# tammypi/flink-siddhi

Measured on AMD Instinct MI355X. Metric: matched-pattern events/sec (whole node) at 1/2/4/8 MI355X + % HBM roofline, higher is better.
Workload: dtype f64+int32+int64

## Files before the change

### flink-siddhi_amd/csrc/cf_kernels.hip

```cpp
#include <hip/hip_runtime.h>

#include "dev_common.h"
#include "kernels.h"
#include "vm.h"

namespace cep {

namespace {

constexpr uint16_t kNoB = 0xffff;
constexpr uint32_t kRolePB = 4;
constexpr int64_t kTolBias = 1ll << 31;
constexpr uint32_t kSkrAlive = 0x8000u;
constexpr int kCfStageBytes = (kCfTile / 8192 * 20 + 36) * 1024;

#ifdef CF_WAVESTAMP
#define CF_STAMP(i) do { } while (0)
#else
#define CF_STAMP(i)                                                                 \
  do {                                                                              \
    if (a.stamps && threadIdx.x == 0 && blockIdx.x < 4096)                          \
      a.stamps[(int64_t)blockIdx.x * 16 + (i)] = __builtin_amdgcn_s_memtime();      \
  } while (0)
#endif
// ... 276 lines not shown
  }
  lds_barrier();
  CF_STAMP(3);
  const uint32_t total = hist[NB];
  const uint32_t nreg = ATL ? hist[P] : total;
  const uint32_t words_t = nreg * RW + (total - nreg);
  const bool staged = words_t <= (uint32_t)(kStageRecs * RW);
  uint64_t* trecs = a.recs + tile * (int64_t)kCfTile * RW;
#pragma unroll
  for (int e = 0; e < E; ++e) {
    if (packed[e] == 0xffffffffu) continue;
    const uint32_t b = (packed[e] >> 13) & 0xfffu;
    const uint32_t role = packed[e] >> 25;
    const uint32_t slot = hist[b] + (packed[e] & 0x1fffu);
    const int64_t dts = (int64_t)tsv[e] - ts_base + (TOL ? kTolBias : 0);
    if (dts < 0) {
      if (TOL) set_err(a.err, ERR_TS_SPAN);
      else if (ATL) *(volatile uint32_t*)a.gate = a.gate_seq;
      else report_descent(a.rows, a.err);
    } else if (dts > 0xffffffffll) {
      set_err(a.err, ERR_TS_SPAN);
    }
    const uint64_t w0 = (uint64_t)(uint32_t)dts | ((uint64_t)(wave * 64 * E + 64 * e + lane) << 32) |
                        ((uint64_t)role << 45) | ((uint64_t)lkey[e] << 48);
    const uint64_t c0 = fc0[e], c1 = fc1[e];
    if (ATL && b >= (uint32_t)P) {
      const uint32_t wd = nreg * RW + (slot - nreg);
      if (staged) stage[wd] = w0;
      else trecs[wd] = w0;
      continue;
    }
    if (staged) {
      stage[slot * RW] = w0;
      if (NW > 0) stage[slot * RW + 1] = c0;
      if (NW > 1) stage[slot * RW + 2] = c1;
    } else {
      uint64_t* g = trecs + (int64_t)slot * RW;
      g[0] = w0;
      if (NW > 0) g[1] = c0;
      if (NW > 1) g[2] = c1;
    }
  }
  for (int i = tid; i <= NB; i += NT) a.tile_off[(int64_t)i * a.ntiles + tile] = (uint16_t)hist[i];
  if (staged) {
    lds_barrier();
    CF_STAMP(4);
    const int64_t words = (int64_t)words_t;
    for (int64_t w = 2 * tid; w < words; w += 2 * NT) {
      if (w + 1 < words) *(uint4*)(trecs + w) = *(const uint4*)(stage + w);
      else trecs[w] = stage[w];
    }
  }
  CF_STAMP(5);
}

#if !defined(CF_UNIT) || CF_UNIT == 1
constexpr int kCfRouteStage = 112 * 1024;
constexpr int kRouteSmallWorld = 8;
__global__ __launch_bounds__(kCfPartThreads, 1) void k_cfroute(CfRouteArgs ca) {
  constexpr int E = kCfItems, NT = kCfPartThreads, NWV = NT / 64;
  const RouteArgs& a = ca.r;
  const PatternArgs& p = a.pat;
  __shared__ uint32_t wcnt[NWV][kMaxWorld];
  __shared__ uint32_t obase[kMaxWorld + 1];
  __shared__ __attribute__((aligned(16))) uint64_t stage[kCfRouteStage / 8];
  const int tid = threadIdx.x, lane = tid & 63, wave = tid >> 6;
  const int world = a.world, wrw = a.wrw;
  const int64_t tile = blockIdx.x;
  for (int i = tid; i < NWV * kMaxWorld; i += NT) wcnt[i / kMaxWorld][i % kMaxWorld] = 0;

  const int64_t r0 = tile * kCfTile + (int64_t)wave * 64 * E + lane;
  const int64_t row0 = a.rows.row0 + r0;
  uint32_t valid = 0;
#pragma unroll
  for (int e = 0; e < E; ++e) valid |= (r0 + 64 * e < a.rows.n ? 1u : 0u) << e;
  uint64_t tsv[E], pv[kPref][E];
#pragma unroll
  for (int e = 0; e < E; ++e) tsv[e] = 0;
  uint32_t is_a = 0, role_a = 0, role_b = 0, role_g = 0;
  uint64_t fkey[E], fc0[E], fc1[E];
#pragma unroll
  for (int e = 0; e < E; ++e) fkey[e] = fc0[e] = fc1[e] = 0;
  if (valid) {
    uint32_t sb[E];
    cf_load_cols<E>(a.rows, ca.pref, ca.ts_slot, row0, valid, tsv, sb, pv);
    uint32_t is_b = 0;
#pragma unroll
    for (int e = 0; e < E; ++e) {
      if ((valid >> e) & 1u) {
        is_a |= ((int)sb[e] == p.a_stream ? 1u : 0u) << e;
        is_b |= ((int)sb[e] == p.b_stream ? 1u : 0u) << e;
      }
    }
    const uint32_t all = (1u << E) - 1u;
    if (is_a) role_a = is_a & (p.f_prog < 0 ? all : eval_terms_regs<E>(p.f_terms, ca.pref.f_slot, a.rows.cols, pv));
    if (is_b) {
      if (p.g_walk_prog >= 0) {
        role_b = is_b;
      } else {
        role_g = is_b & (p.g_raw_prog < 0 ? all : eval_terms_regs<E>(p.g_terms, ca.pref.g_slot, a.rows.cols, pv));
        role_b = p.tolerant ? is_b : role_g;
      }
    }
    if (p.nrec_a > 0 || p.nrec_b > 0)
      pick_carried<E>(pv, p.nrec_a > 0 ? ca.pref.reca_slot[0] : -1, p.nrec_b > 0 ? ca.pref.recb_slot[0] : -1,
                      is_a, fc0);
// ... 1126 lines not shown
  }
  const int np = a.pref.n <= 2 ? 2 : a.pref.n;
  switch (a.cf.nw * 8 + np) {
    case 0 * 8 + 2: hipLaunchKernelGGL((k_cfpart<0, false, 2, true>), g, b, dyn, s, a); break;
    case 0 * 8 + 3: hipLaunchKernelGGL((k_cfpart<0, false, 3, true>), g, b, dyn, s, a); break;
    case 0 * 8 + 4: hipLaunchKernelGGL((k_cfpart<0, false, 4, true>), g, b, dyn, s, a); break;
    case 1 * 8 + 2: hipLaunchKernelGGL((k_cfpart<1, false, 2, true>), g, b, dyn, s, a); break;
    case 1 * 8 + 3: hipLaunchKernelGGL((k_cfpart<1, false, 3, true>), g, b, dyn, s, a); break;
    case 1 * 8 + 4: hipLaunchKernelGGL((k_cfpart<1, false, 4, true>), g, b, dyn, s, a); break;
    case 2 * 8 + 2: hipLaunchKernelGGL((k_cfpart<2, false, 2, true>), g, b, dyn, s, a); break;
    case 2 * 8 + 3: hipLaunchKernelGGL((k_cfpart<2, false, 3, true>), g, b, dyn, s, a); break;
    default: hipLaunchKernelGGL((k_cfpart<2, false, 4, true>), g, b, dyn, s, a); break;
  }
}
#endif

template <int NW, bool ATL>
static void cf_part_local(const CfPartArgs& a, int64_t ntiles, hipStream_t s) {
  const int P = 1 << a.pat.buckets_log2;
  const size_t dyn = ((size_t)(P + a.nhot + 1) * 4 + 15) & ~(size_t)15;
  const dim3 g((unsigned)ntiles), b(kCfPartThreads);
  const int np = a.pref.n <= 2 ? 2 : a.pref.n;
  switch (np) {
    case 2: hipLaunchKernelGGL((k_cfpart<NW, false, 2, false, ATL>), g, b, dyn, s, a); break;
    case 3: hipLaunchKernelGGL((k_cfpart<NW, false, 3, false, ATL>), g, b, dyn, s, a); break;
    default: hipLaunchKernelGGL((k_cfpart<NW, false, 4, false, ATL>), g, b, dyn, s, a); break;
  }
}
void cf_part_et0(const CfPartArgs&, int64_t, hipStream_t);
void cf_part_et1(const CfPartArgs&, int64_t, hipStream_t);
void cf_part_et2(const CfPartArgs&, int64_t, hipStream_t);
void cf_part_atl0(const CfPartArgs&, int64_t, hipStream_t);
void cf_part_atl1(const CfPartArgs&, int64_t, hipStream_t);
void cf_part_atl2(const CfPartArgs&, int64_t, hipStream_t);
#if !defined(CF_UNIT) || CF_UNIT == 9
void cf_part_et0(const CfPartArgs& a, int64_t n, hipStream_t s) { cf_part_local<0, false>(a, n, s); }
#endif
#if !defined(CF_UNIT) || CF_UNIT == 10
void cf_part_et1(const CfPartArgs& a, int64_t n, hipStream_t s) { cf_part_local<1, false>(a, n, s); }
#endif
#if !defined(CF_UNIT) || CF_UNIT == 11
void cf_part_et2(const CfPartArgs& a, int64_t n, hipStream_t s) { cf_part_local<2, false>(a, n, s); }
#endif
#if !defined(CF_UNIT) || CF_UNIT == 12
void cf_part_atl0(const CfPartArgs& a, int64_t n, hipStream_t s) { cf_part_local<0, true>(a, n, s); }
#endif
#if !defined(CF_UNIT) || CF_UNIT == 13
void cf_part_atl1(const CfPartArgs& a, int64_t n, hipStream_t s) { cf_part_local<1, true>(a, n, s); }
#endif
#if !defined(CF_UNIT) || CF_UNIT == 14
void cf_part_atl2(const CfPartArgs& a, int64_t n, hipStream_t s) { cf_part_local<2, true>(a, n, s); }
#endif

#if !defined(CF_UNIT) || CF_UNIT == 1
void launch_cf_partition(const CfPartArgs& a, int64_t ntiles, hipStream_t s) {
  if (a.in_recs || (a.pat.tolerant && !a.atol)) {
    cf_part_tol(a, ntiles, s);
    return;
  }
  switch (a.cf.nw) {
    case 0: a.atol ? cf_part_atl0(a, ntiles, s) : cf_part_et0(a, ntiles, s); break;
    case 1: a.atol ? cf_part_atl1(a, ntiles, s) : cf_part_et1(a, ntiles, s); break;
    default: a.atol ? cf_part_atl2(a, ntiles, s) : cf_part_et2(a, ntiles, s); break;
  }
}
#endif

template <int NW, bool KR, bool TOL, bool ATL, bool LEAN>
static void launch_cf_walk_nc(const CfWalkArgs& a, int nbuckets, hipStream_t s) {
  const dim3 g((unsigned)nbuckets), b(kCfWalkThreads);
  switch (a.pat.slot_words - 2) {
    case 0: hipLaunchKernelGGL((k_cfwalk<NW, KR, 0, TOL, ATL, LEAN>), g, b, 0, s, a); break;
    case 1: hipLaunchKernelGGL((k_cfwalk<NW, KR, 1, TOL, ATL, LEAN>), g, b, 0, s, a); break;
    default: hipLaunchKernelGGL((k_cfwalk<NW, KR, 2, TOL, ATL, LEAN>), g, b, 0, s, a); break;
  }
}

template <bool KR, bool TOL, bool ATL, bool LEAN>
static void cf_walk_mode(const CfWalkArgs& a, int nbuckets, hipStream_t s) {
  switch (a.cf.nw) {
    case 0: launch_cf_walk_nc<0, KR, TOL, ATL, LEAN>(a, nbuckets, s); break;
    case 1: launch_cf_walk_nc<1, KR, TOL, ATL, LEAN>(a, nbuckets, s); break;
    default: launch_cf_walk_nc<2, KR, TOL, ATL, LEAN>(a, nbuckets, s); break;
  }
}
#define CF_WALK_UNIT(name, KR, TOL, ATL, LEAN) \
  void name(const CfWalkArgs& a, int nb, hipStream_t s) { cf_walk_mode<KR, TOL, ATL, LEAN>(a, nb, s); }
#if !defined(CF_UNIT) || CF_UNIT == 2
CF_WALK_UNIT(cf_walk_et0, false, false, false, false)
#endif
#if !defined(CF_UNIT) || CF_UNIT == 3
CF_WALK_UNIT(cf_walk_et1, true, false, false, false)
#endif
#if !defined(CF_UNIT) || CF_UNIT == 4
CF_WALK_UNIT(cf_walk_tol0, false, true, false, false)
#endif
#if !defined(CF_UNIT) || CF_UNIT == 5
CF_WALK_UNIT(cf_walk_tol1, true, true, false, false)
#endif
#if !defined(CF_UNIT) || CF_UNIT == 6
CF_WALK_UNIT(cf_walk_atl0, false, false, true, false)
#endif
#if !defined(CF_UNIT) || CF_UNIT == 7
CF_WALK_UNIT(cf_walk_atl1, true, false, true, false)
#endif
#if !defined(CF_UNIT) || CF_UNIT == 15
CF_WALK_UNIT(cf_walk_et0c, false, false, false, true)
#endif
#if !defined(CF_UNIT) || CF_UNIT == 16
CF_WALK_UNIT(cf_walk_et1c, true, false, false, true)
// ... 34 lines not shown
```

### flink-siddhi_amd/csrc/engine.cpp

```cpp
#include <hip/hip_runtime.h>

#include <algorithm>
#include <cstdio>
#include <cstdlib>
#include <cstring>
#include <memory>
#include <numeric>
#include <string>
#include <unordered_map>
#include <vector>

#include "../../include/cep.h"
#include "frontend.h"
#include "kernels.h"

using namespace cep;

namespace {

struct DevBuf {
  void* p = nullptr;
  size_t bytes = 0;
};

// ... 150 lines not shown
  hipStream_t stream = nullptr;
  hipStream_t side = nullptr;
  hipEvent_t in_ready = nullptr;
  hipEvent_t ext_ready = nullptr;
  hipEvent_t out_ready = nullptr;
  hipStream_t rstream = nullptr;
  hipEvent_t r_ready = nullptr;
  hipEvent_t r_host = nullptr;
  bool enabled = true;
  std::string last_error;
  std::vector<std::string> dict;
  std::unordered_map<std::string, int32_t> dict_index;
  DevBuf code, konst;
  std::vector<OutStream> outs;
  std::vector<PatternRT> pats;
  std::vector<MqRT> mqs;
  std::vector<char> in_mq;
  DevBuf tile_state, ticket, err;
  DevBuf route_arena, route_tcount, route_toffs, route_dcount;
  DevBuf rerr;
  DevBuf stamps;
  DevBuf str_hash;
  HostBuf flush_words;
  DevBuf out_counts;
  DevBuf ostats;
  DevBuf okeys[2], oidx[2], otemp;
  DevBuf rr_col[kMaxCols], rr_ts, rr_stream, rr_seq;
  struct ViewStage {
    DevBuf stream, col[kMaxCols];
  };
  std::vector<std::vector<ViewStage>> views;
  struct HostSlot {
    HostBuf pinned;
    DevBuf dev;
    hipEvent_t dma_done = nullptr, free = nullptr;
    bool used = false;
  } hs[2];
  int hs_next = 0;
  hipStream_t copy = nullptr;
  struct Reorder {
    int input = -1;
    bool has_stream = false;
    int64_t n = 0, cap = 0;
    int64_t released_max = INT64_MIN;
    DevBuf col[kMaxCols], ts, stream;
    DevBuf out[kMaxCols], ots, ostream;
    DevBuf keys, idx_in, idx_out, temp, bound;
  } ro;
  int64_t events_in = 0, matches_out = 0, batches = 0, late_events = 0;
  int64_t last_ts = INT64_MIN;
  DevBuf last_ts_dev;
  bool force_tolerant = false;
  bool seq_poison = false;
  int64_t launches[16] = {0};
  double kernel_ms[16] = {0};
  int64_t kernel_timed[16] = {0};
  std::vector<TimedLaunch> timed;
  std::vector<hipEvent_t> event_pool;
  std::vector<std::unique_ptr<char[]>> name_store;
};

namespace {

void set_err(char* err, size_t errlen, const std::string& m) {
  if (err && errlen) {
    std::snprintf(err, errlen, "%s", m.c_str());
  }
}

int fail(cep_app* a, int code, const std::string& m) {
  if (a) a->last_error = m;
  return code;
}

hipEvent_t pool_event(cep_app* a) {
  if (!a->event_pool.empty()) {
    hipEvent_t e = a->event_pool.back();
    a->event_pool.pop_back();
    return e;
  }
  hipEvent_t e;
  hipEventCreate(&e);
  return e;
}

struct LaunchTimer {
  cep_app* a;
  int kind;
  hipStream_t st;
  hipEvent_t s = nullptr;
  LaunchTimer(cep_app* app, int k, hipStream_t on = nullptr)
      : a(app), kind(k), st(on ? on : app->stream) {
    const bool timed = a->opt.profile > 0 && a->launches[k] % a->opt.profile == 0;
    a->launches[k]++;
    if (timed) {
      s = pool_event(a);
      hipEventRecord(s, st);
    }
  }
  ~LaunchTimer() {
    if (s) {
      hipEvent_t e = pool_event(a);
      hipEventRecord(e, st);
      a->timed.push_back({kind, s, e});
    }
  }
// ... 563 lines not shown
        for (size_t sl = 0; sl < pc.size(); ++sl)
          if (pc[sl] == mc.tl.t[i].col) mc.slot[i] = (int32_t)sl;
    hipMemcpy(g.dconds.p, g.conds.data(), g.conds.size() * sizeof(MqCond), hipMemcpyHostToDevice);
    hipMemcpy(g.du.p, g.units.data(), g.units.size() * sizeof(MqUnit), hipMemcpyHostToDevice);
  }
  return CEP_OK;
}

int create_runtime(cep_app* a) {
  const CompiledApp& app = a->app;
  if (hipSetDevice(a->opt.device) != hipSuccess)
    return fail(a, CEP_E_DEVICE, "no HIP device " + std::to_string(a->opt.device));
  hipDeviceProp_t prop;
  if (hipGetDeviceProperties(&prop, a->opt.device) != hipSuccess)
    return fail(a, CEP_E_DEVICE, "hipGetDeviceProperties failed");
  if (std::string(prop.gcnArchName).find("gfx950") == std::string::npos)
    return fail(a, CEP_E_DEVICE, std::string("libcep is built for gfx950, device is ") +
                                     prop.gcnArchName);
  if (hipStreamCreateWithFlags(&a->stream, hipStreamNonBlocking) != hipSuccess ||
      hipStreamCreateWithFlags(&a->side, hipStreamNonBlocking) != hipSuccess ||
      hipEventCreateWithFlags(&a->in_ready, hipEventDisableTiming) != hipSuccess ||
      hipEventCreateWithFlags(&a->ext_ready, hipEventDisableTiming) != hipSuccess ||
      hipEventCreateWithFlags(&a->out_ready, hipEventDisableTiming) != hipSuccess ||
      hipStreamCreateWithFlags(&a->copy, hipStreamNonBlocking) != hipSuccess ||
      hipStreamCreateWithFlags(&a->rstream, hipStreamNonBlocking) != hipSuccess ||
      hipEventCreateWithFlags(&a->r_ready, hipEventDisableTiming) != hipSuccess ||
      hipEventCreateWithFlags(&a->r_host, hipEventDisableTiming) != hipSuccess)
    return fail(a, CEP_E_DEVICE, "hipStreamCreate failed");
  size_t cb = std::max<size_t>(app.code.size(), 1) * sizeof(Ins);
  size_t kb = std::max<size_t>(app.konst.size(), 1) * 8;
  if (!dev_ensure(&a->code, cb, a->stream, false) || !dev_ensure(&a->konst, kb, a->stream, false) ||
      !dev_ensure(&a->err, 64, a->stream, false) || !dev_ensure(&a->rerr, 64, a->stream, false) ||
      !dev_ensure(&a->ticket, 64, a->stream, false))
    return fail(a, CEP_E_DEVICE, "out of device memory (plan)");
  if (!app.code.empty())
    hipMemcpy(a->code.p, app.code.data(), app.code.size() * sizeof(Ins), hipMemcpyHostToDevice);
  if (!app.konst.empty())
    hipMemcpy(a->konst.p, app.konst.data(), app.konst.size() * 8, hipMemcpyHostToDevice);
  hipMemset(a->err.p, 0, 64);
  hipMemset(a->rerr.p, 0, 64);
  if (!dev_ensure(&a->out_counts, std::max<size_t>(app.outputs.size(), 1) * 8, a->stream, false))
    return fail(a, CEP_E_DEVICE, "out of device memory");
  hipMemset(a->out_counts.p, 0, std::max<size_t>(app.outputs.size(), 1) * 8);
  for (auto& sd : app.outputs) {
    OutStream o;
    o.id = sd.id;
    for (auto& at : sd.attrs) o.types.push_back(at.type);
    o.cols.resize(sd.attrs.size());
    o.count = (unsigned long long*)a->out_counts.p + a->outs.size();
    o.write_seq = !(a->opt.omit_seq && !a->opt.ordered_output);
    a->outs.push_back(std::move(o));
    if (const char* e = std::getenv("CEP_SEQ_POISON")) a->seq_poison = std::atoi(e) != 0;
  }
  {
    const int rc = build_mq_groups(a);
    if (rc) return rc;
  }
  for (size_t qi = 0; qi < app.queries.size(); ++qi) {
    const Query& q = app.queries[qi];
    if (q.kind != Q_PATTERN && q.kind != Q_AGG) continue;
    if (a->in_mq[qi]) continue;
    const bool agg = q.kind == Q_AGG;
    const bool win = agg && q.win_kind != WIN_NONE;
    const int S = agg ? 1 : a->opt.pending_slots;
    PatternRT rt;
    rt.q = (int)qi;
    PatternArgs& p = rt.pa;
    if (win) {
      if (q.win_global && a->opt.ts_order != 1)
        return fail(a, CEP_E_UNSUPPORTED,
                    "group by with #window.time outside a partition is not supported with ts_order = 0: Siddhi's "
                    "window spans every group, and one window per group equals it only for non-decreasing "
                    "timestamps (set ts_order = 1, or partition the query)");
      if (q.win_kind == WIN_LENGTH && q.win_param > kWinMaxRing)
        return fail(a, CEP_E_CAPACITY, "#window.length(" + std::to_string(q.win_param) + ") exceeds the capacity of " +
                                           std::to_string(kWinMaxRing) + " window rows per key");
      WinArgs& w = rt.win;
      w.kind = q.win_kind;
      w.param = q.win_param;
      w.ring = q.win_kind == WIN_LENGTH ? (int)q.win_param : a->opt.pending_slots;
      w.nval = 0;
      for (size_t i = 0; i < q.aggs.size(); ++i) {
        w.agg_val[i] = -1;
        if (q.aggs[i].word < 0) continue;
        for (int v = 0; v < w.nval; ++v)
          if (w.val_word[v] == q.aggs[i].word) w.agg_val[i] = v;
        if (w.agg_val[i] < 0) {
          w.val_word[w.nval] = q.aggs[i].word;
          w.agg_val[i] = w.nval++;
        }
      }
      w.entry_words = w.nval + (q.win_kind == WIN_TIME ? 1 : 0);
      rt.win_vm = q.having.valid();
      for (auto& it : q.select) rt.win_vm |= it.src == SRC_VM;
    }
    p.a_stream = q.a_stream;
    p.b_stream = q.b_stream;
    p.f_prog = q.f.off;
    p.g_raw_prog = q.g_raw.off;
    p.g_walk_prog = q.g_walk.off;
    p.f_terms = q.f_terms;
    p.g_terms = q.g_terms;
    p.every = q.every ? 1 : 0;
    p.within = q.within;
    p.key_col_a = q.key_col_a;
    p.key_col_b = q.key_col_b;
// ... 396 lines not shown
  for (int i = pf.n; i < kPref; ++i) pf.col[i] = pf.col[0];
  for (int i = 0; i < nf; ++i) down(pf.f_slot[i]);
  for (int i = 0; i < ng; ++i) down(pf.g_slot[i]);
  for (int w = 0; w < 2; ++w) {
    down(pa->cf.a_slot[w]);
    down(pa->cf.b_slot[w]);
  }
  down(pf.key_slot);
  pa->ts_slot = -1;
}

int run_pattern_cf(cep_app* a, PatternRT& rt, const Query& q, OutStream& o,
                   const RowsArgs& rows_all, const CfPlan& cf,
                   const uint64_t* in_recs = nullptr, int in_rec_words = 0, bool tol = false) {
  const int P = 1 << rt.pa.buckets_log2;
  const bool hot_ok = rt.hot;
  static const bool overlap = std::getenv("CEP_OVERLAP") != nullptr;
  hipStream_t side = overlap ? a->side : a->stream;
  if (overlap) {
    hipEventRecord(a->in_ready, a->stream);
    hipStreamWaitEvent(a->side, a->in_ready, 0);
  }
  constexpr int64_t kHotProbeRows = 1 << 20;
  for (int64_t r0 = 0, step = 0; r0 < rows_all.n; r0 += step) {
    const int b = rt.cur;
    rt.cur ^= 1;
    const bool probe = hot_ok && !rt.hot_on && !rt.hot_probed;
    step = std::min<int64_t>(probe ? std::min<int64_t>(kHotProbeRows, rt.cf_chunk) : rt.cf_chunk, rows_all.n - r0);
    RowsArgs rows = rows_all;
    rows.row0 = rows_all.row0 + r0;
    rows.n = step;
    if (r0 > 0) rows.prev_ts = INT64_MIN;
    const int64_t ntiles = (rows.n + kCfTile - 1) / kCfTile;
    CfPartArgs pa{};
    pa.rows = rows;
    pa.pref = rt.pref;
    pa.ts_slot = -1;
    pa.in_recs = in_recs;
    pa.in_rec_words = in_rec_words;
    for (int i = 0; i < rt.pref.n && !in_recs; ++i)
      if (rows.cols.p[rt.pref.col[i]] == (const void*)rows.ts && rows.cols.t[rt.pref.col[i]] == T_LONG)
        pa.ts_slot = i;
    pa.pat = rt.pa;
    pa.pat.tolerant = tol ? 1 : 0;
    pa.cf = cf;
    cf_drop_ts_slot(&pa);
    pa.chunk_base = (int64_t*)rt.chunk_base[b].p;
    pa.recs = (uint64_t*)rt.cf_recs[b].p;
    pa.tile_off = (uint16_t*)rt.cf_toff[b].p;
    pa.ntiles = (int32_t)ntiles;
    pa.err = (unsigned int*)a->err.p;
    static const int stagger = std::getenv("CEP_CF_STAGGER") ? std::atoi(std::getenv("CEP_CF_STAGGER")) : 1280;
    pa.stagger = ntiles >= 4 * kCfStaggerBlocks ? stagger : 0;
    pa.pool_cursor = overlap ? nullptr : (unsigned long long*)rt.pool_cur.p;
    if (overlap) hipMemsetAsync(rt.pool_cur.p, 0, 8, a->stream);
    if (a->stamps.p) pa.stamps = (uint64_t*)a->stamps.p + 4096 * 16;
    const bool hot = hot_ok;
    if (hot && !rt.hot_on && *(volatile uint32_t*)rt.hot_active_host.p > 0) {
      const int rw = 1 + cf.nw;
      const int64_t cc = rt.cf_chunk, ntmax = cc / kCfTile;
      rt.hot_blocks = (int)((cc + kHotBlock - 1) / kHotBlock);
      const bool ok = dev_ensure(&rt.hot_gbase, (kCfHotMax + 1) * 4, a->stream, false) &&
                      dev_ensure(&rt.hoff, (size_t)kCfHotMax * ntmax * 4, a->stream, false) &&
                      dev_ensure(&rt.harr, (size_t)cc * rw * 8, a->stream, false) &&
                      dev_ensure(&rt.hrow, (size_t)cc * 4, a->stream, false) &&
                      dev_ensure(&rt.hnb, (size_t)cc * 4, a->stream, false) &&
                      dev_ensure(&rt.bsum, (size_t)rt.hot_blocks * 16, a->stream, false) &&
                      dev_ensure(&rt.bcnt, (size_t)rt.hot_blocks * 4, a->stream, false) &&
                      dev_ensure(&rt.boff, (size_t)rt.hot_blocks * 4, a->stream, false) &&
                      dev_ensure(&rt.hcm, kCfHotMax * 3 * 4, a->stream, false) &&
                      dev_ensure(&rt.hobase, 64, a->stream, false) &&
                      dev_ensure(&rt.htmn, (size_t)cc * 4, a->stream, false) &&
                      dev_ensure(&rt.htmx, (size_t)cc * 4, a->stream, false) &&
                      dev_ensure(&rt.hflag, (size_t)cc, a->stream, false) &&
                      dev_ensure(&rt.btol, (size_t)rt.hot_blocks * 12, a->stream, false);
      if (!ok) return fail(a, CEP_E_DEVICE, "out of device memory (hot-key arenas)");
      rt.hot_on = true;
    }
    const bool divert = hot && rt.hot_on;
    pa.hot_id = divert ? (const uint16_t*)rt.hot_id.p : nullptr;
    pa.nhot = divert ? kCfHotMax : 0;
    static const bool no_atol = std::getenv("CEP_NO_ATOL") != nullptr;
    const bool atol = tol && !in_recs && !divert && rt.atol_ok && rt.hwm.p && !no_atol &&
                      (2 << rt.pa.buckets_log2) <= kCfMaxBuckets && q.a_stream != q.b_stream;
    uint32_t gseq = 0;
    if (tol && rt.hwm.p) {
      const int par = (int)(rt.tol_chunks++ & 1);
      pa.hwm_rd = (const unsigned long long*)rt.hwm.p + (par ^ 1) * 64;
      pa.hwm_wr = (unsigned long long*)rt.hwm.p + par * 64;
    }
    if (atol) {
      if (++rt.atol_seq == 0) ++rt.atol_seq;
      gseq = rt.atol_seq;
      pa.gate = (uint32_t*)rt.atol_gate.p;
      pa.gate_seq = gseq;
    }
    if (overlap && rt.used[b]) hipStreamWaitEvent(side, rt.walk_done[b], 0);
    if (overlap && hot && rt.used[b ^ 1]) hipStreamWaitEvent(side, rt.walk_done[b ^ 1], 0);
    if (atol) {
      CfPartArgs aa = pa;
      aa.atol = 1;
      aa.pat.tolerant = 0;
      aa.nhot = P;
      aa.hot_id = nullptr;
      LaunchTimer t(a, CEP_K_CF_PARTITION, side);
      launch_cf_partition(aa, ntiles, side);
    }
    {
      LaunchTimer t(a, atol ? CEP_K_OTHER : CEP_K_CF_PARTITION, side);
      launch_cf_partition(pa, ntiles, side);
    }
    if (overlap) {
      hipEventRecord(rt.part_done[b], side);
      hipStreamWaitEvent(a->stream, rt.part_done[b], 0);
    }
    CfWalkArgs wa{};
    wa.pat = pa.pat;
    wa.cf = cf;
    wa.recs = pa.recs;
    wa.tile_off = pa.tile_off;
    wa.ntiles = (int32_t)ntiles;
    wa.chunk_base = (const int64_t*)rt.chunk_base[b].p;
    wa.khdr = (uint32_t*)rt.khdr.p;
    wa.kslot = (uint64_t*)rt.kslot.p;
    wa.kstride = rt.kstride;
    wa.kext = (uint64_t*)rt.kext.p;
    wa.pool_rd = (const uint64_t*)rt.pool[rt.pool_side].p;
    wa.pool_wr = (uint64_t*)rt.pool[rt.pool_side ^ 1].p;
    wa.pool_cursor = (unsigned long long*)rt.pool_cur.p;
    wa.pool_cap = (uint64_t)rt.pool_cap;
    wa.key_rev = rt.sparse ? (const uint64_t*)rt.krev.p : nullptr;
    wa.out = out_args(o, q);
    wa.err = pa.err;
    HotArgs ha{};
    if (hot) {
      ha.pat = pa.pat;
      ha.cf = cf;
      ha.recs = pa.recs;
      ha.tile_off = pa.tile_off;
      ha.ntiles = (int32_t)ntiles;
      ha.chunk_base = (const int64_t*)rt.chunk_base[b].p;
      ha.hot_id = (uint16_t*)rt.hot_id.p;
      ha.hot_key = (int32_t*)rt.hot_key.p;
      ha.hot_m = (uint32_t*)rt.hot_m.p;
      ha.hot_gbase = (uint32_t*)rt.hot_gbase.p;
      ha.hoff = (uint32_t*)rt.hoff.p;
      ha.cand = (uint64_t*)rt.cand.p;
      ha.ncand = (uint32_t*)rt.ncand.p;
      ha.cand_cap = kCfHotMax * 4;
      ha.thresh = rt.hot_thresh;
      ha.harr = (uint64_t*)rt.harr.p;
      ha.hrow = (uint32_t*)rt.hrow.p;
      ha.hnb = (uint32_t*)rt.hnb.p;
      ha.bsum = (uint32_t*)rt.bsum.p;
      ha.bcnt = (uint32_t*)rt.bcnt.p;
      ha.boff = (uint32_t*)rt.boff.p;
      ha.hcm = (uint32_t*)rt.hcm.p;
      ha.obase = (unsigned long long*)rt.hobase.p;
      ha.htmn = (uint32_t*)rt.htmn.p;
      ha.htmx = (uint32_t*)rt.htmx.p;
      ha.hflag = (uint8_t*)rt.hflag.p;
      ha.btol = (uint32_t*)rt.btol.p;
// ... 2273 lines not shown
```

### flink-siddhi_amd/csrc/kernels.h

```cpp
#pragma once
#include <hip/hip_runtime.h>

#include <cstdint>

#include "plan.h"

namespace cep {

struct ColSet {
  const void* p[kMaxCols];
  int32_t t[kMaxCols];
  int32_t n;
};

struct RowsArgs {
  ColSet cols;
  const int64_t* ts;
  const uint8_t* stream;
  int32_t input;
  int64_t row0;
  int64_t n;
  int64_t seq0;
  int64_t prev_ts;
  const int64_t* seq;
// ... 215 lines not shown
  OutArgs out;
  unsigned int* err;
};

#ifndef CF_TILE_ROWS
#define CF_TILE_ROWS 8192
#endif
constexpr int kCfItems = 8;
constexpr int kCfPartThreads = CF_TILE_ROWS / kCfItems;
constexpr int kCfTile = CF_TILE_ROWS;
constexpr int kCfWalkThreads = 512;
constexpr int kCfWindow = 2048;
constexpr int kCfMaxKeys = 512;
constexpr int kCfMaxTiles = (32 << 20) / kCfTile;
constexpr int kCfMaxBuckets = 4096;
constexpr int kCfMaxCaps = 2;
constexpr int kCfMaxOut = 8;

struct CfPlan {
  int32_t nw;
  int32_t a_slot[2], b_slot[2];
  int32_t a_log[2], b_log[2];
  int32_t cap_phys[kMaxCaps];
  int32_t bcol_phys[kMaxCaps];
};

constexpr int kCfHotMax = 1024;
constexpr int kHotBlock = 2048;
constexpr uint16_t kNotHot = 0xffff;

struct CfPartArgs {
  RowsArgs rows;
  const uint16_t* hot_id;
  int32_t nhot;
  PrefPlan pref;
  int32_t ts_slot;
  const uint64_t* in_recs;
  int32_t in_rec_words;
  PatternArgs pat;
  CfPlan cf;
  int64_t* chunk_base;
  uint64_t* recs;
  uint16_t* tile_off;
  int32_t ntiles;
  uint64_t* stamps;
  unsigned int* err;
  int32_t atol;
  uint32_t* gate;
  uint32_t gate_seq;
  const unsigned long long* hwm_rd;
  unsigned long long* hwm_wr;
  unsigned long long* pool_cursor;
  int32_t stagger;
};
constexpr int kCfStaggerBlocks = 256;

struct CfWalkArgs {
  PatternArgs pat;
  CfPlan cf;
  const uint64_t* recs;
  const uint16_t* tile_off;
  int32_t ntiles;
  const int64_t* chunk_base;
  uint32_t* khdr;
  uint64_t* kslot;
  int64_t kstride;
  uint64_t* kext;
  const uint64_t* pool_rd;
  uint64_t* pool_wr;
  unsigned long long* pool_cursor;
  uint64_t pool_cap;
  const uint64_t* key_rev;
  const uint16_t* hot_id;
  uint64_t* hot_cand;
  uint32_t* hot_ncand;
  uint32_t hot_thresh;
  OutArgs out;
  const uint64_t* in_seq;
  int32_t in_rec_words;
  uint64_t* stamps;
  int32_t ablate;
  unsigned int* err;
  int32_t atol;
  const uint32_t* gate;
  uint32_t gate_seq;
};

struct HotArgs {
  PatternArgs pat;
  CfPlan cf;
  const uint64_t* recs;
  const uint16_t* tile_off;
  int32_t ntiles;
  const int64_t* chunk_base;
  uint16_t* hot_id;
  int32_t* hot_key;
  uint32_t* hot_m;
  uint32_t* hot_gbase;
  uint32_t* hoff;
  uint64_t* cand;
  uint32_t* ncand;
  uint32_t cand_cap;
  uint32_t thresh;
  uint64_t* harr;
  uint32_t* hrow;
  uint32_t* hnb;
// ... 153 lines not shown
  int32_t nphys;
  int32_t lmap[kMqMaxCarry];
  const uint64_t* recs;
  const uint16_t* tile_off;
  int32_t ntiles;
  int32_t buckets_log2;
  int32_t kpb;
  int32_t key_stride, key_offset;
  const int64_t* chunk_base;
  const int64_t* in_seq;
  uint64_t* state;
  int64_t kstride;
  int64_t words;
  uint64_t* stamps;
  int32_t ablate;
  unsigned int* err;
};

constexpr int kDeriveProds = 4;
constexpr int kDerivePref = 6;
constexpr int kDeriveThreads = 256;
constexpr int kDeriveRows = 8;
struct DeriveProd {
  int32_t src, dst;
  int32_t filter_prog;
  TermList terms;
  int32_t fslot[kMaxTerms];
  int32_t item_src[kMaxCols];
  int32_t item_prog[kMaxCols];
  int32_t item_slot[kMaxCols];
};
struct DeriveArgs {
  RowsArgs rows;
  VmArgs vm;
  int32_t nprod;
  DeriveProd prod[kDeriveProds];
  uint8_t* stream_out;
  int32_t ncols;
  void* col_out[kMaxCols];
  int32_t out_type[kMaxCols];
  int32_t own_col[kMaxCols];
  int32_t own_slot[kMaxCols];
  int32_t npref;
  int32_t pcol[kDerivePref];
  int32_t col_slot[kMaxCols];
  int32_t vec;
  unsigned int* err;
};
void launch_derive(const DeriveArgs& a, bool vm, bool rowwise, hipStream_t s);

void launch_mq_partition(const MqPartArgs& a, hipStream_t s);
void launch_mq_walk(const MqWalkArgs& a, int nbuckets, hipStream_t s);
void launch_cf_partition(const CfPartArgs& a, int64_t ntiles, hipStream_t s);
void launch_cf_walk(const CfWalkArgs& a, int nbuckets, hipStream_t s);
void launch_keymap(const KeyMapArgs& a, hipStream_t s);
void launch_route_keys(const RouteKeyArgs& a, hipStream_t s);
void launch_hot_match(const HotArgs& a, hipStream_t s);
void launch_hot_update(const HotArgs& a, int diverted, hipStream_t s);
void launch_filter(const FilterArgs& a, int64_t ntiles, bool vm, hipStream_t s);
void launch_filterc(const FilterArgs& a, int64_t ntiles, hipStream_t s);
int filterc_rows_per_tile();
void launch_partition(const PartArgs& a, int64_t ntiles, bool vm, hipStream_t s);
void launch_route(const RouteArgs& a, int64_t ntiles, bool vm, uint32_t* toffs,
                  unsigned long long* dcount, uint64_t* out, hipStream_t s);
void launch_route_collect(const RouteArgs& a, int64_t ntiles, uint32_t* toffs,
                          unsigned long long* dcount, uint64_t* out, hipStream_t s);
void launch_route_pad(const RouteArgs& a, const unsigned long long* dcount, uint64_t* out, hipStream_t s);
void launch_route_check(const uint64_t* segs, int world, int64_t seg_cap, int wrw, int row_mode, unsigned int* err,
                        hipStream_t s);
void launch_route_rows(const RowRouteArgs& a, int64_t ntiles, uint32_t* toffs,
                       unsigned long long* dcount, uint64_t* out, hipStream_t s);
void launch_unpack_rows(const RowUnpackArgs& a, hipStream_t s);
void launch_cf_route(const CfRouteArgs& a, int64_t ntiles, hipStream_t s);
void launch_walk(const WalkArgs& a, int nbuckets, bool vm, hipStream_t s);
void launch_winwalk(const WinArgs& a, int nbuckets, bool vm, hipStream_t s);
size_t reorder_temp_bytes(int64_t n);
int reorder_sort(void* temp, size_t temp_bytes, const int64_t* keys_in, int64_t* keys_out, int32_t* idx_in,
                 int32_t* idx_out, int64_t n, hipStream_t s);
void launch_upper_bound(const int64_t* sorted, int64_t n, int64_t wm, int64_t* out3, hipStream_t s);
void launch_gather(const void* src, void* dst, const int32_t* perm, int64_t first, int64_t n, int width,
                   hipStream_t s);
void launch_seq_stats(const int64_t* seq, const unsigned long long* count, int64_t cap, unsigned long long* out3,
                      hipStream_t s);
size_t order_temp_bytes(int64_t n);
int order_sort(void* temp, size_t temp_bytes, const int64_t* seq, int64_t n, int64_t lo, int bits, void* keys_a,
               void* keys_b, int32_t* idx_a, int32_t* idx_b, hipStream_t s);
void launch_generate(int64_t first, int64_t n, uint64_t seed, int64_t keys,
                     int64_t rate, int64_t t0, int single_stream, int32_t* key,
                     int64_t* ts, uint8_t* stream, int32_t* id, double* price,
                     hipStream_t s);

constexpr int kFilterThreads = 512;
constexpr int kFilterItems = 16;
constexpr int kPartThreads = 512;
constexpr int kPartItems = 4;
constexpr int kWalkThreads = 512;
constexpr int kWalkWindow = 1024;
constexpr int kWalkMaxTiles = 8192;
constexpr int kWalkMaxKeys = 512;
constexpr int kWalkCapLds = 2;
constexpr int kMaxPending = 16;

}
```

### flink-siddhi_amd/flink_siddhi/_lib.py

```python
from __future__ import annotations

import ctypes as C
import os
from pathlib import Path

_HERE = Path(__file__).resolve().parent
LIB_PATH = Path(os.environ.get("CEP_LIB", str(_HERE.parent / "libcep.so")))

CEP_OK = 0
CEP_E_PARSE = 1
CEP_E_UNDEFINED_STREAM = 2
CEP_E_DUPLICATED_STREAM = 3
CEP_E_UNSUPPORTED = 4
CEP_E_ARG = 5
CEP_E_DEVICE = 6
CEP_E_CAPACITY = 7
CEP_E_STATE = 8

INT, LONG, FLOAT, DOUBLE, BOOL, STRING, OBJECT = range(7)
TYPE_NAMES = {INT: "int", LONG: "long", FLOAT: "float", DOUBLE: "double",
              BOOL: "bool", STRING: "string", OBJECT: "object"}
NUMPY_DTYPES = {INT: "int32", LONG: "int64", FLOAT: "float32",
                DOUBLE: "float64", BOOL: "uint8", STRING: "int32"}

(K_FILTER, K_PARTITION, K_WALK, K_ROUTE, K_ORDER, K_AGG, K_OTHER, K_CF_PARTITION, K_CF_WALK, K_HOT,
 K_MQ_PARTITION, K_MQ_WALK) = range(12)


class SiddhiError(RuntimeError):
    code = -1


class SiddhiAppCreationException(SiddhiError):
    code = CEP_E_PARSE


class UndefinedStreamException(SiddhiError):
    code = CEP_E_UNDEFINED_STREAM


class DuplicatedStreamException(SiddhiError):
    code = CEP_E_DUPLICATED_STREAM


class UnsupportedPlanException(SiddhiError):
    code = CEP_E_UNSUPPORTED


class CepDeviceError(SiddhiError):
    code = CEP_E_DEVICE


class CepCapacityError(SiddhiError):
    code = CEP_E_CAPACITY


class CepStateError(SiddhiError):
    code = CEP_E_STATE


_EXC = {CEP_E_PARSE: SiddhiAppCreationException,
        CEP_E_UNDEFINED_STREAM: UndefinedStreamException,
        CEP_E_DUPLICATED_STREAM: DuplicatedStreamException,
        CEP_E_UNSUPPORTED: UnsupportedPlanException,
        CEP_E_ARG: ValueError, CEP_E_DEVICE: CepDeviceError,
        CEP_E_CAPACITY: CepCapacityError, CEP_E_STATE: CepStateError}


def raise_for(code: int, msg: str):
    if code == CEP_OK:
        return
    exc = _EXC.get(code, SiddhiError)
    raise exc(msg)


class cep_attr(C.Structure):
    _fields_ = [("name", C.c_char * 64), ("type", C.c_int32)]


# ... 134 lines not shown
```

### include/cep.h

```cpp
#ifndef CEP_H_
#define CEP_H_

#include <stddef.h>
#include <stdint.h>

#ifdef __cplusplus
extern "C" {
#endif

enum {
  CEP_OK = 0,
  CEP_E_PARSE = 1,
  CEP_E_UNDEFINED_STREAM = 2,
  CEP_E_DUPLICATED_STREAM = 3,
  CEP_E_UNSUPPORTED = 4,
  CEP_E_ARG = 5,
  CEP_E_DEVICE = 6,
  CEP_E_CAPACITY = 7,
  CEP_E_STATE = 8
};

typedef enum {
  CEP_INT = 0, CEP_LONG = 1, CEP_FLOAT = 2, CEP_DOUBLE = 3, CEP_BOOL = 4,
  CEP_STRING = 5, CEP_OBJECT = 6
// ... 13 lines not shown
  int32_t profile;
  int32_t ordered_output;
  int32_t key_stride;
  int32_t key_offset;
  int32_t pending_pool_log2;
  int32_t sparse_keys;
  int32_t late_policy;
  int32_t omit_seq;
  int32_t ts_order;
  int32_t reserved[2];
} cep_options;

void cep_default_options(cep_options* opt);

typedef struct cep_app cep_app;

typedef struct {
  int64_t n;
  const int64_t* ts;
  const uint8_t* stream;
  int32_t input;
  int32_t ncols;
  const void* const* cols;
  int32_t on_device;
} cep_batch;

typedef struct {
  const char* stream_id;
  int64_t n;
  int32_t ncols;
  const int64_t* ts;
  const int64_t* seq;
  const void* const* cols;
} cep_rows;

typedef void (*cep_emit_fn)(void* user, const cep_rows* rows);

typedef struct {
  int64_t events_in;
  int64_t matches_out;
  int64_t batches;
  int64_t kernel_launches[16];
  double kernel_ms[16];
  int64_t kernel_timed[16];
  int64_t late_events;
  int64_t hot_keys;
} cep_stats_t;

enum {
  CEP_K_FILTER = 0, CEP_K_PARTITION = 1, CEP_K_WALK = 2, CEP_K_ROUTE = 3,
  CEP_K_ORDER = 4, CEP_K_AGG = 5, CEP_K_OTHER = 6,
  CEP_K_CF_PARTITION = 7, CEP_K_CF_WALK = 8,
  CEP_K_HOT = 9,
  CEP_K_MQ_PARTITION = 10, CEP_K_MQ_WALK = 11
};


int cep_validate(const char* plan, char* err, size_t errlen);

int cep_plan_schema(const char* plan, const char* stream_id, cep_attr* out,
                    int cap, int* n, char* err, size_t errlen);


cep_app* cep_create(const char* plan, const cep_options* opt, char* err,
                    size_t errlen);

void cep_destroy(cep_app* app);

int cep_stream_schema(cep_app* app, const char* stream_id, cep_attr* out,
                      int cap, int* n);

int cep_input(cep_app* app, const char* stream_id);

int cep_set_callback(cep_app* app, const char* out_id, cep_emit_fn fn,
                     void* user);

int cep_send_batch(cep_app* app, const cep_batch* batch);

int cep_buffer_batch(cep_app* app, const cep_batch* batch);

int cep_watermark(cep_app* app, int64_t mark);

int64_t cep_buffered(cep_app* app);

int cep_flush(cep_app* app);

int cep_output_device(cep_app* app, const char* out_id, cep_rows* rows);

int cep_reset_output(cep_app* app);

int cep_snapshot(cep_app* app, uint8_t** buf, size_t* len);
int cep_restore(cep_app* app, const uint8_t* buf, size_t len);
void cep_free(void* p);

int cep_set_enabled(cep_app* app, int enabled);

int cep_stream_wait(cep_app* app, void* hip_stream);

int cep_stream_signal(cep_app* app, void* hip_stream);

int32_t cep_dict_intern(cep_app* app, const char* s);
const char* cep_dict_lookup(cep_app* app, int32_t id);

int cep_stats(cep_app* app, cep_stats_t* out);
const char* cep_last_error(cep_app* app);

int cep_record_words(cep_app* app);
// ... 57 lines not shown
```

Measured before the change: 52.01 billion.

## Add multi-workgroup-per-CU partition kernel with smaller LDS pending buffer

Adds a new CF partition kernel that uses 512 threads and about 80KB of LDS so that several workgroups can be resident per CU (launch bounds 4). It processes each tile in sub-parts, stages records in a compact LDS pending buffer, and then scatters them in bucket order through an index permutation. If a tile's record count exceeds the buffer, it falls back to a direct global-atomic scatter that recomputes the whole tile. The new kernel becomes the default for the non-tolerant, non-hot path, and an env var restores the old kernel. The aim is better latency hiding through higher occupancy, at the cost of a second pass on overflowing tiles and indirect LDS reads.

```diff
diff --git a/flink-siddhi_amd/csrc/cf_kernels.hip b/flink-siddhi_amd/csrc/cf_kernels.hip
--- a/flink-siddhi_amd/csrc/cf_kernels.hip
+++ b/flink-siddhi_amd/csrc/cf_kernels.hip
@@ -352,6 +352,233 @@
     }
   }
   CF_STAMP(5);
+}
+
+constexpr int kCf2Threads = 512;
+template <int NP>
+constexpr int cf2_items() { return NP > 3 ? kCfItems / 2 : kCfItems; }
+constexpr int kCf2LdsBytes = 80 * 1024;
+template <int RW>
+constexpr int cf2_pending() {
+  return ((kCf2LdsBytes - (kCfMaxBuckets + 4) * 4 - 64) / (8 * RW + 6)) & ~7;
+}
+
+__device__ __forceinline__ const CfPartArgs& cf2_args() {
+  auto kp = __builtin_amdgcn_kernarg_segment_ptr();
+  asm volatile("" : "+s"(kp));
+  return *(const CfPartArgs*)kp;
+}
+
+template <int NW, int NP, bool DIRECT>
+__device__ __forceinline__ void cf2_half(int64_t tile, int h, bool full, int64_t ts_base, uint32_t* hist,
+                                         uint64_t* pend, uint32_t* pbr, uint32_t* s_cnt, uint64_t* trecs) {
+  constexpr int E = cf2_items<NP>(), RW = 1 + NW;
+  constexpr uint32_t CAP = (uint32_t)cf2_pending<RW>();
+  const CfPartArgs& a = cf2_args();
+  const PatternArgs& p = a.pat;
+  const int tid = threadIdx.x, lane = tid & 63, wave = tid >> 6;
+  const int lg = p.buckets_log2;
+  const int P = 1 << lg;
+  const uint32_t trow = (uint32_t)(h * kCf2Threads * E + wave * 64 * E + lane);
+  const int64_t r0 = tile * kCfTile + trow;
+  const int64_t row0 = a.rows.row0 + r0;
+  uint32_t valid = 0;
+#pragma unroll
+  for (int e = 0; e < E; ++e) valid |= (r0 + 64 * e < a.rows.n ? 1u : 0u) << e;
+  uint32_t role_a = 0, role_b = 0, keep = 0;
+  uint32_t bk[E], dts[E];
+  uint64_t fc0[E], fc1[E];
+#pragma unroll
+  for (int e = 0; e < E; ++e) {
+    bk[e] = dts[e] = 0;
+    fc0[e] = fc1[e] = 0;
+  }
+  if (valid) {
+    uint64_t tsv[E];
+    uint64_t pv[NP][E];
+    uint32_t sb[E];
+    int64_t before_full = 0;
+    if (full) cf_load_cols_full<E, NP>(a.rows, a.pref, a.ts_slot, row0, tsv, sb, pv, &before_full);
+    else cf_load_cols<E, NP>(a.rows, a.pref, a.ts_slot, row0, valid, tsv, sb, pv);
+    uint32_t is_a = 0, is_b = 0;
+#pragma unroll
+    for (int e = 0; e < E; ++e) {
+      if ((valid >> e) & 1u) {
+        is_a |= ((int)sb[e] == p.a_stream ? 1u : 0u) << e;
+        is_b |= ((int)sb[e] == p.b_stream ? 1u : 0u) << e;
+      }
+    }
+    if (p.within >= 0) {
+      int64_t before;
+      if (full) before = row0 > 0 ? before_full : batch_prev_ts(a.rows);
+      else before = row0 > 0 ? a.rows.ts[row0 - 1] : batch_prev_ts(a.rows);
+      bool bad = false;
+#pragma unroll
+      for (int e = 0; e < E; ++e) {
+        const uint64_t up = __shfl_up(tsv[e], 1, 64);
+        const uint64_t last = e > 0 ? __shfl(tsv[e > 0 ? e - 1 : 0], 63, 64) : 0ull;
+        const int64_t prev = lane > 0 ? (int64_t)up : (e > 0 ? (int64_t)last : before);
+        if ((valid >> e) & 1u) bad |= (int64_t)tsv[e] < prev;
+      }
+      if (bad) report_descent(a.rows, a.err);
+    }
+    uint32_t neg = 0, big = 0;
+#pragma unroll
+    for (int e = 0; e < E; ++e) {
+      const int64_t d = (int64_t)tsv[e] - ts_base;
+      neg |= (d < 0 ? 1u : 0u) << e;
+      big |= (d > 0xffffffffll ? 1u : 0u) << e;
+      dts[e] = (uint32_t)d;
+    }
+    const uint32_t all = (1u << E) - 1u;
+    if (is_a) role_a = is_a & (p.f_prog < 0 ? all : eval_terms_regs<E, NP>(p.f_terms, a.pref.f_slot, a.rows.cols, pv));
+    if (is_b) role_b = is_b & (p.g_raw_prog < 0 ? all : eval_terms_regs<E, NP>(p.g_terms, a.pref.g_slot, a.rows.cols, pv));
+#pragma unroll
+    for (int e = 0; e < E; ++e) {
+      if (!(((role_a | role_b) >> e) & 1u)) continue;
+      const int64_t key = a.pref.key_slot >= 0 ? (int64_t)pv[0][e] : 0;
+      const int64_t kfield = shard_key(key, p.key_stride, p.key_offset);
+      if (kfield < 0 || kfield >= p.key_capacity) {
+        set_err(a.err, ERR_KEY_RANGE);
+        continue;
+      }
+      keep |= 1u << e;
+      bk[e] = (uint32_t)(kfield & (P - 1)) | ((uint32_t)(kfield >> lg) << 12);
+      if ((neg >> e) & 1u) report_descent(a.rows, a.err);
+      else if ((big >> e) & 1u) set_err(a.err, ERR_TS_SPAN);
+    }
+    if (NW > 0) pick_carried<E, NP>(pv, a.cf.a_slot[0], a.cf.b_slot[0], role_a, fc0);
+    if (NW > 1) pick_carried<E, NP>(pv, a.cf.a_slot[1], a.cf.b_slot[1], role_a, fc1);
+  }
+  uint32_t slot = 0;
+  if (!DIRECT) {
+    const uint32_t nk = (uint32_t)__popc(keep);
+    const uint32_t incl = wave_incl_scan(nk);
+    uint32_t base = 0;
+    if (lane == 63) base = atomicAdd(s_cnt, incl);
+    base = (uint32_t)__shfl((int)base, 63, 64);
+    slot = base + incl - nk;
+  }
+#pragma unroll
+  for (int e = 0; e < E; ++e) {
+    if (!((keep >> e) & 1u)) continue;
+    const uint32_t role = ((role_a >> e) & 1u) * ROLE_A | ((role_b >> e) & 1u) * ROLE_B;
+    const uint32_t bucket = bk[e] & 0xfffu;
+    const uint64_t w0 = (uint64_t)dts[e] | ((uint64_t)(trow + 64 * e) << 32) | ((uint64_t)role << 45) |
+                        ((uint64_t)(bk[e] >> 12) << 48);
+    const uint32_t rank = atomicAdd(&hist[bucket], 1u);
+    if (DIRECT) {
+      uint64_t* g = trecs + (int64_t)rank * RW;
+      g[0] = w0;
+      if (NW > 0) g[1] = fc0[e];
+      if (NW > 1) g[2] = fc1[e];
+    } else {
+      if (slot < CAP) {
+        pend[slot * RW] = w0;
+        if (NW > 0) pend[slot * RW + 1] = fc0[e];
+        if (NW > 1) pend[slot * RW + 2] = fc1[e];
+        pbr[slot] = (bucket << 13) | rank;
+      }
+      ++slot;
+    }
+  }
+}
+
+template <int NW, int NP>
+__global__ __launch_bounds__(kCf2Threads, 4) void k_cfpart2(CfPartArgs a) {
+  constexpr int NT = kCf2Threads, RW = 1 + NW;
+  constexpr int NPART = kCfTile / (NT * cf2_items<NP>());
+  static_assert(NPART * NT * cf2_items<NP>() == kCfTile && kCfItems == 8, "a tile is whole parts");
+  constexpr int CAP = cf2_pending<RW>();
+  __shared__ uint32_t scratch[NT / 64 + 1];
+  __shared__ uint32_t s_cnt;
+  __shared__ __attribute__((aligned(16))) uint64_t pend[CAP * RW];
+  __shared__ uint32_t pbr[CAP];
+  __shared__ uint16_t sidx[CAP];
+  extern __shared__ __attribute__((aligned(16))) uint32_t hist[];
+  const int tid = threadIdx.x;
+  const int64_t tile = xcd_tile(blockIdx.x, a.ntiles);
+  if (a.stagger > 0 && blockIdx.x < 2 * kCfStaggerBlocks) {
+    const uint64_t t0 = __builtin_amdgcn_s_memtime();
+    const uint64_t d = (uint64_t)((blockIdx.x >> 3) & 63u) * (uint64_t)a.stagger / 2;
+    while (__builtin_amdgcn_s_memtime() - t0 < d) __builtin_amdgcn_s_sleep(8);
+  }
+  const int P = 1 << a.pat.buckets_log2;
+  CF_STAMP(0);
+  for (int i = tid; i <= P; i += NT) hist[i] = 0;
+  if (tid == 0) s_cnt = 0;
+  const int64_t ts_base = a.rows.ts[a.rows.row0];
+  if (tile == 0 && tid == 0) {
+    if (a.pool_cursor) *a.pool_cursor = 0ull;
+    a.chunk_base[0] = ts_base;
+    a.chunk_base[1] = a.rows.seq0 + a.rows.row0;
+  }
+  const bool full = (tile + 1) * (int64_t)kCfTile <= a.rows.n;
+  uint64_t* trecs = a.recs + tile * (int64_t)kCfTile * RW;
+  lds_barrier();
+#pragma unroll 1
+  for (int h = 0; h < NPART; ++h) {
+    cf2_half<NW, NP, false>(tile, h, full, ts_base, hist, pend, pbr, &s_cnt, trecs);
+    if (h == 0) CF_STAMP(1);
+  }
+  CF_STAMP(2);
+  lds_barrier();
+  {
+    constexpr int MAXPER = kCfMaxBuckets / NT;
+    const int per = (P + NT - 1) / NT;
+    uint32_t c[MAXPER];
+    uint32_t sum = 0;
+#pragma unroll
+    for (int i = 0; i < MAXPER; ++i) {
+      const int idx = tid * per + i;
+      c[i] = (i < per && idx < P) ? hist[idx] : 0u;
+      sum += c[i];
+    }
+    uint32_t total;
+    uint32_t off = bscan<NT>(sum, scratch, &total);
+#pragma unroll
+    for (int i = 0; i < MAXPER; ++i) {
+      const int idx = tid * per + i;
+      if (i < per && idx < P) {
+        hist[idx] = off;
+        off += c[i];
+      }
+    }
+    if (tid == 0) hist[P] = total;
+  }
+  lds_barrier();
+  CF_STAMP(3);
+  const uint32_t total = hist[P];
+  for (int i = tid; i <= P; i += NT) a.tile_off[(int64_t)i * a.ntiles + tile] = (uint16_t)hist[i];
+  if (total <= (uint32_t)CAP) {
+    for (uint32_t i = tid; i < total; i += NT) {
+      const uint32_t br = pbr[i];
+      sidx[hist[br >> 13] + (br & 0x1fffu)] = (uint16_t)i;
+    }
+    lds_barrier();
+    CF_STAMP(4);
+    if (RW == 2) {
+      for (uint32_t s = tid; s < total; s += NT)
+        *(uint4*)(trecs + 2 * (int64_t)s) = *(const uint4*)(pend + 2 * (uint32_t)sidx[s]);
+    } else {
+      const uint32_t words = total * RW;
+      for (uint32_t w = 2 * tid; w < words; w += 2 * NT) {
+        const uint64_t x0 = pend[(uint32_t)sidx[w / RW] * RW + w % RW];
+        if (w + 1 < words) {
+          const uint64_t x1 = pend[(uint32_t)sidx[(w + 1) / RW] * RW + (w + 1) % RW];
+          *(uint4*)(trecs + w) = make_uint4((uint32_t)x0, (uint32_t)(x0 >> 32), (uint32_t)x1, (uint32_t)(x1 >> 32));
+        } else {
+          trecs[w] = x0;
+        }
+      }
+    }
+    CF_STAMP(5);
+  } else {
+    lds_barrier();
+#pragma unroll 1
+    for (int h = 0; h < NPART; ++h) cf2_half<NW, NP, true>(tile, h, full, ts_base, hist, pend, pbr, &s_cnt, trecs);
+    CF_STAMP(6);
+  }
 }
 
 #if !defined(CF_UNIT) || CF_UNIT == 1
@@ -1584,10 +1811,47 @@
 void cf_part_atl2(const CfPartArgs& a, int64_t n, hipStream_t s) { cf_part_local<2, true>(a, n, s); }
 #endif
 
+template <int NW>
+static void cf_part_2wg(const CfPartArgs& a, int64_t ntiles, hipStream_t s) {
+  const int P = 1 << a.pat.buckets_log2;
+  const size_t dyn = ((size_t)(P + 1) * 4 + 15) & ~(size_t)15;
+  const dim3 g((unsigned)ntiles), b(kCf2Threads);
+  const int np = a.pref.n <= 2 ? 2 : a.pref.n;
+  switch (np) {
+    case 2: hipLaunchKernelGGL((k_cfpart2<NW, 2>), g, b, dyn, s, a); break;
+    case 3: hipLaunchKernelGGL((k_cfpart2<NW, 3>), g, b, dyn, s, a); break;
+    default: hipLaunchKernelGGL((k_cfpart2<NW, 4>), g, b, dyn, s, a); break;
+  }
+}
+void cf_part_2wg0(const CfPartArgs&, int64_t, hipStream_t);
+void cf_part_2wg1(const CfPartArgs&, int64_t, hipStream_t);
+void cf_part_2wg2(const CfPartArgs&, int64_t, hipStream_t);
+#if !defined(CF_UNIT) || CF_UNIT == 21
+void cf_part_2wg0(const CfPartArgs& a, int64_t n, hipStream_t s) { cf_part_2wg<0>(a, n, s); }
+#endif
+#if !defined(CF_UNIT) || CF_UNIT == 22
+void cf_part_2wg1(const CfPartArgs& a, int64_t n, hipStream_t s) { cf_part_2wg<1>(a, n, s); }
+#endif
+#if !defined(CF_UNIT) || CF_UNIT == 23
+void cf_part_2wg2(const CfPartArgs& a, int64_t n, hipStream_t s) { cf_part_2wg<2>(a, n, s); }
+#endif
+
 #if !defined(CF_UNIT) || CF_UNIT == 1
+bool cf_partition_2wg(const CfPartArgs& a) {
+  return !a.in_recs && !a.pat.tolerant && !a.atol && a.nhot == 0 && !a.one_wg;
+}
+
 void launch_cf_partition(const CfPartArgs& a, int64_t ntiles, hipStream_t s) {
   if (a.in_recs || (a.pat.tolerant && !a.atol)) {
     cf_part_tol(a, ntiles, s);
+    return;
+  }
+  if (cf_partition_2wg(a)) {
+    switch (a.cf.nw) {
+      case 0: cf_part_2wg0(a, ntiles, s); break;
+      case 1: cf_part_2wg1(a, ntiles, s); break;
+      default: cf_part_2wg2(a, ntiles, s); break;
+    }
     return;
   }
   switch (a.cf.nw) {
diff --git a/flink-siddhi_amd/csrc/engine.cpp b/flink-siddhi_amd/csrc/engine.cpp
--- a/flink-siddhi_amd/csrc/engine.cpp
+++ b/flink-siddhi_amd/csrc/engine.cpp
@@ -226,6 +226,7 @@
   DevBuf last_ts_dev;
   bool force_tolerant = false;
   bool seq_poison = false;
+  bool cf_one_wg = false;
   int64_t launches[16] = {0};
   double kernel_ms[16] = {0};
   int64_t kernel_timed[16] = {0};
@@ -895,6 +896,7 @@
     a->outs.push_back(std::move(o));
     if (const char* e = std::getenv("CEP_SEQ_POISON")) a->seq_poison = std::atoi(e) != 0;
   }
+  if (const char* e = std::getenv("CEP_CF_PART")) a->cf_one_wg = std::atoi(e) == 1;
   {
     const int rc = build_mq_groups(a);
     if (rc) return rc;
@@ -1397,6 +1399,7 @@
     pa.err = (unsigned int*)a->err.p;
     static const int stagger = std::getenv("CEP_CF_STAGGER") ? std::atoi(std::getenv("CEP_CF_STAGGER")) : 1280;
     pa.stagger = ntiles >= 4 * kCfStaggerBlocks ? stagger : 0;
+    pa.one_wg = a->cf_one_wg ? 1 : 0;
     pa.pool_cursor = overlap ? nullptr : (unsigned long long*)rt.pool_cur.p;
     if (overlap) hipMemsetAsync(rt.pool_cur.p, 0, 8, a->stream);
     if (a->stamps.p) pa.stamps = (uint64_t*)a->stamps.p + 4096 * 16;
@@ -1453,6 +1456,7 @@
     }
     {
       LaunchTimer t(a, atol ? CEP_K_OTHER : CEP_K_CF_PARTITION, side);
+      if (cf_partition_2wg(pa)) a->launches[CEP_K_CF_PARTITION_2WG]++;
       launch_cf_partition(pa, ntiles, side);
     }
     if (overlap) {
diff --git a/flink-siddhi_amd/csrc/kernels.h b/flink-siddhi_amd/csrc/kernels.h
--- a/flink-siddhi_amd/csrc/kernels.h
+++ b/flink-siddhi_amd/csrc/kernels.h
@@ -291,6 +291,7 @@
   unsigned long long* hwm_wr;
   unsigned long long* pool_cursor;
   int32_t stagger;
+  int32_t one_wg;
 };
 constexpr int kCfStaggerBlocks = 256;
 
@@ -550,6 +551,7 @@
 void launch_mq_partition(const MqPartArgs& a, hipStream_t s);
 void launch_mq_walk(const MqWalkArgs& a, int nbuckets, hipStream_t s);
 void launch_cf_partition(const CfPartArgs& a, int64_t ntiles, hipStream_t s);
+bool cf_partition_2wg(const CfPartArgs& a);
 void launch_cf_walk(const CfWalkArgs& a, int nbuckets, hipStream_t s);
 void launch_keymap(const KeyMapArgs& a, hipStream_t s);
 void launch_route_keys(const RouteKeyArgs& a, hipStream_t s);
diff --git a/flink-siddhi_amd/flink_siddhi/_lib.py b/flink-siddhi_amd/flink_siddhi/_lib.py
--- a/flink-siddhi_amd/flink_siddhi/_lib.py
+++ b/flink-siddhi_amd/flink_siddhi/_lib.py
@@ -24,7 +24,7 @@
                 DOUBLE: "float64", BOOL: "uint8", STRING: "int32"}
 
 (K_FILTER, K_PARTITION, K_WALK, K_ROUTE, K_ORDER, K_AGG, K_OTHER, K_CF_PARTITION, K_CF_WALK, K_HOT,
- K_MQ_PARTITION, K_MQ_WALK) = range(12)
+ K_MQ_PARTITION, K_MQ_WALK, K_CF_PARTITION_2WG) = range(13)
 
 
 class SiddhiError(RuntimeError):
diff --git a/include/cep.h b/include/cep.h
--- a/include/cep.h
+++ b/include/cep.h
@@ -89,7 +89,8 @@
   CEP_K_ORDER = 4, CEP_K_AGG = 5, CEP_K_OTHER = 6,
   CEP_K_CF_PARTITION = 7, CEP_K_CF_WALK = 8,
   CEP_K_HOT = 9,
-  CEP_K_MQ_PARTITION = 10, CEP_K_MQ_WALK = 11
+  CEP_K_MQ_PARTITION = 10, CEP_K_MQ_WALK = 11,
+  CEP_K_CF_PARTITION_2WG = 12
 };
 
 
```

New measurement: 53.75 billion (median of 6 runs). 1.03x the previous value.
